# ewrfcas/MVSFormer

Hardware: AMD Instinct MI355X
Metric: depth maps/sec @1536x1152 N=5 D=192 (higher is better)
Workload: dtype f32

## Files before the change

mvsformer_amd/csrc/conv3d_x3_small.hip:

```cpp
#include <stdlib.h>

#include "conv_common.h"
#include "split3.h"

namespace {
using namespace mvsconv;
using mvsx3::bf16x8;
using mvsx3::mfma6;
using mvsx3::Split3;
using mvsx3::split3;

#ifndef SMALL_PF
#define SMALL_PF 4
#endif
constexpr int PF = SMALL_PF;

struct SmallArgs {
    const float* x;
    const bf16x8* wp;
    const float* scale;
    const float* shift;
    const float* residual;
    float* y;
    int B, Cin, Cout, Di, Hi, Wi, Do, Ho, Wo, stride, relu;
    int tiles_w, items;
};

__host__ __device__ inline int steps_of(int nblocks) { return (nblocks + 3) >> 2; }
__host__ __device__ inline int ntap(int p) { return p ? 2 : 1; }
__host__ __device__ inline void dtap(int p, int j, int* k, int* off) {
    if (!p) { *k = 1; *off = 0; }
    else if (j == 0) { *k = 2; *off = 0; }
    else { *k = 0; *off = 1; }
}
__host__ __device__ inline int deconv_class_step0(int KQ, int cls) {
    int s = 0;
    for (int c = 0; c < cls; ++c) s += steps_of(ntap(c >> 2) * ntap((c >> 1) & 1) * ntap(c & 1) * KQ);
    return s;
}
__host__ __device__ inline int deconv_total_steps(int KQ) { return deconv_class_step0(KQ, 8); }

__global__ void small_pack_kernel(const float* __restrict__ w, int Cin, int Cout, int transposed, bf16x8* __restrict__ out, int total) {
    const int idx = blockIdx.x * blockDim.x + threadIdx.x;
    if (idx >= total) return;
    const int KQ = Cin / 8;
    const int lane = idx & 63, term = (idx >> 6) % 3, gstep = idx / 192;
    const int n = lane & 15, kb = lane >> 4;
    bf16x8 v;
    if (!transposed) {
        const int STEPS = steps_of(27 * KQ), ct = gstep / STEPS, step = gstep % STEPS;
        const int q = 4 * step + kb, co = ct * 16 + n;
#pragma unroll
        for (int e = 0; e < 8; ++e) {
            float f = 0.0f;
            if (q < 27 * KQ && co < Cout) f = w[((size_t)co * Cin + (q % KQ) * 8 + e) * 27 + q / KQ];
            v[e] = mvsx3::split3_term(f, term);
        }
    } else {
        const int TOTAL = deconv_total_steps(KQ), ct = gstep / TOTAL;
        int rem = gstep % TOTAL, cls = 0;
        while (cls < 7 && rem >= deconv_class_step0(KQ, cls + 1) - deconv_class_step0(KQ, cls)) {
            rem -= deconv_class_step0(KQ, cls + 1) - deconv_class_step0(KQ, cls);
            ++cls;
        }
        const int pd = cls >> 2, ph = (cls >> 1) & 1, pw = cls & 1;
        const int nh = ntap(ph), nw = ntap(pw), nt = ntap(pd) * nh * nw;
        const int q = 4 * rem + kb, co = ct * 16 + n;
        int kd = 0, kh = 0, kw = 0, o;
        if (q < nt * KQ) {
            const int t = q / KQ;
            dtap(pd, t / (nh * nw), &kd, &o);
            dtap(ph, (t / nw) % nh, &kh, &o);
            dtap(pw, t % nw, &kw, &o);
        }
#pragma unroll
        for (int e = 0; e < 8; ++e) {
            float f = 0.0f;
            if (q < nt * KQ && co < Cout) f = w[((size_t)((q % KQ) * 8 + e) * Cout + co) * 27 + (kd * 3 + kh) * 3 + kw];
            v[e] = mvsx3::split3_term(f, term);
        }
    }
    out[idx] = v;
}

struct WFrag { bf16x8 t[3]; };
__device__ __forceinline__ WFrag load_w(const bf16x8* wk) {
    WFrag f;
#pragma unroll
    for (int t = 0; t < 3; ++t) f.t[t] = wk[t * 64];
    return f;
}
struct AFrag { float f[8]; };
__device__ __forceinline__ AFrag load_a(rsrc_t xin, unsigned voff, unsigned plane_bytes) {
    AFrag a;
#pragma unroll
    for (int e = 0; e < 8; ++e) a.f[e] = buf_load(xin, voff, (unsigned)e * plane_bytes);
    return a;
}
__device__ __forceinline__ f32x4 step_mfma(const AFrag& a, const WFrag& w, f32x4 c) {
    const Split3 s = split3(a.f);
    return mfma6(s.h, s.m, s.l, w.t[0], w.t[1], w.t[2], c);
}

template <bool TRANSPOSED, int KS>
__global__ __launch_bounds__(256) void x3_small_kernel(const SmallArgs a) {
    const int lane = threadIdx.x & 63;
    const int wave = (int)__builtin_amdgcn_readfirstlane(threadIdx.x >> 6);
    const int item = KS == 1 ? blockIdx.x * 4 + wave : blockIdx.x;
    const int ks = KS == 1 ? 0 : wave;
    if (item >= a.items) return;
    __shared__ f32x4 red[KS == 1 ? 1 : 2 * 4 * 64];
    const int m = lane & 15, kb = lane >> 4;
    const int KQ = a.Cin >> 3, kq_shift = 31 - __builtin_clz(KQ);
    const int CT = (a.Cout + 15) >> 4;
    int r = item;
    const int wt = r % a.tiles_w; r /= a.tiles_w;
    const int oh = r % a.Ho; r /= a.Ho;
    const int od = r % a.Do; r /= a.Do;
    const int ct = r % CT, b = r / CT;
    const size_t HWi = (size_t)a.Hi * a.Wi, DHWi = (size_t)a.Di * HWi, HWo = (size_t)a.Ho * a.Wo;
    const rsrc_t xin = make_rsrc(a.x + (size_t)b * a.Cin * DHWi, (unsigned)((size_t)a.Cin * DHWi * 4));
    const unsigned plane_bytes = (unsigned)(DHWi * 4);
    const int co = ct * 16 + m;
    const float sc = (a.scale && co < a.Cout) ? a.scale[co] : 1.0f, sh = (a.shift && co < a.Cout) ? a.shift[co] : 0.0f;
    auto act = [&](float v) {
        v = a.scale ? fmaf(v, sc, sh) : v + sh;
        return a.relu ? fmaxf(v, 0.0f) : v;
    };

    if constexpr (!TRANSPOSED) {
        const int S = a.stride, nblk = 27 * KQ, nsteps = steps_of(nblk);
        const bf16x8* wk = a.wp + (size_t)ct * nsteps * 192 + lane;
        const int ow = wt * 16 + m;
        const int zb = od * S - 1, yb = oh * S - 1, xb = ow * S - 1;
        auto a_off = [&](int s) -> unsigned {
            const int q = 4 * s + kb, t = q >> kq_shift, oct = q & (KQ - 1);
            const int kd = t / 9, kh = (t / 3) % 3, kw = t % 3;
            const int z = zb + kd, y = yb + kh, x = xb + kw;
            const bool ok = q < nblk && ow < a.Wo && (unsigned)z < (unsigned)a.Di && (unsigned)y < (unsigned)a.Hi && (unsigned)x < (unsigned)a.Wi;
            return ok ? ((((unsigned)(oct * 8) * (unsigned)a.Di + (unsigned)z) * (unsigned)a.Hi + (unsigned)y) * (unsigned)a.Wi + (unsigned)x) * 4u : OOB;
        };
        f32x4 acc = {0.f, 0.f, 0.f, 0.f};
        AFrag ar[PF];
        WFrag wr[PF];
#pragma unroll
        for (int i = 0; i < PF; ++i)
            if (ks + i * KS < nsteps) {
                ar[i] = load_a(xin, a_off(ks + i * KS), plane_bytes);
                wr[i] = load_w(wk + (size_t)(ks + i * KS) * 192);
            }
        for (int s0 = ks; s0 < nsteps; s0 += PF * KS) {
#pragma unroll
            for (int i = 0; i < PF; ++i) {
                const int s = s0 + i * KS;
                if (s < nsteps) {
                    acc = step_mfma(ar[i], wr[i], acc);
                    if (s + PF * KS < nsteps) {
                        ar[i] = load_a(xin, a_off(s + PF * KS), plane_bytes);
                        wr[i] = load_w(wk + (size_t)(s + PF * KS) * 192);
                    }
                }
            }
        }
        if constexpr (KS > 1) {
            red[wave * 64 + lane] = acc;
            __syncthreads();
            if (wave != 0) return;
            acc = ((red[lane] + red[64 + lane]) + red[128 + lane]) + red[192 + lane];
        }
        const int ow0 = wt * 16 + kb * 4;
        if (co < a.Cout && ow0 < a.Wo) {
            const size_t o = ((size_t)(b * a.Cout + co) * a.Do + od) * HWo + (size_t)oh * a.Wo + ow0;
            f32x4 v;
#pragma unroll
            for (int i = 0; i < 4; ++i) v[i] = act(acc[i]);
            if ((a.Wo & 3) == 0) {
                if (a.residual) v += *reinterpret_cast<const f32x4*>(a.residual + o);
                *reinterpret_cast<f32x4*>(a.y + o) = v;
            } else {
#pragma unroll
                for (int i = 0; i < 4; ++i)
                    if (ow0 + i < a.Wo) a.y[o + i] = a.residual ? v[i] + a.residual[o + i] : v[i];
            }
        }
    } else {
        const int pd = od & 1, ph = oh & 1, id0 = od >> 1, ih0 = oh >> 1;
        const int iw = wt * 16 + m;
        const int nd = ntap(pd), nh = ntap(ph);
        const int TOTAL = deconv_total_steps(KQ);
        f32x4 acc[2];
#pragma unroll
        for (int pw = 0; pw < 2; ++pw) {
            const int nw = ntap(pw), nblk = nd * nh * nw * KQ, nsteps = steps_of(nblk);
            const int cls = pd * 4 + ph * 2 + pw;
            const bf16x8* wk = a.wp + ((size_t)ct * TOTAL + deconv_class_step0(KQ, cls)) * 192 + lane;
            auto a_off = [&](int s) -> unsigned {
                const int q = 4 * s + kb, t = q >> kq_shift, oct = q & (KQ - 1);
                const int td = t / (nh * nw), th = (t / nw) % nh, tw = t % nw;
                const int z = id0 + (pd ? td : 0), y = ih0 + (ph ? th : 0), x = iw + (pw ? tw : 0);
                const bool ok = q < nblk && z < a.Di && y < a.Hi && x < a.Wi;
                return ok ? ((((unsigned)(oct * 8) * (unsigned)a.Di + (unsigned)z) * (unsigned)a.Hi + (unsigned)y) * (unsigned)a.Wi + (unsigned)x) * 4u : OOB;
            };
            f32x4 c = {0.f, 0.f, 0.f, 0.f};
            AFrag ar[PF];
            WFrag wr[PF];
#pragma unroll
            for (int i = 0; i < PF; ++i)
                if (ks + i * KS < nsteps) {
                    ar[i] = load_a(xin, a_off(ks + i * KS), plane_bytes);
                    wr[i] = load_w(wk + (size_t)(ks + i * KS) * 192);
                }
            for (int s0 = ks; s0 < nsteps; s0 += PF * KS) {
#pragma unroll
                for (int i = 0; i < PF; ++i) {
                    const int s = s0 + i * KS;
                    if (s < nsteps) {
                        c = step_mfma(ar[i], wr[i], c);
                        if (s + PF * KS < nsteps) {
                            ar[i] = load_a(xin, a_off(s + PF * KS), plane_bytes);
                            wr[i] = load_w(wk + (size_t)(s + PF * KS) * 192);
                        }
                    }
                }
            }
            acc[pw] = c;
        }
        if constexpr (KS > 1) {
            red[wave * 64 + lane] = acc[0];
            red[256 + wave * 64 + lane] = acc[1];
            __syncthreads();
            if (wave != 0) return;
            acc[0] = ((red[lane] + red[64 + lane]) + red[128 + lane]) + red[192 + lane];
            acc[1] = ((red[256 + lane] + red[320 + lane]) + red[384 + lane]) + red[448 + lane];
        }
        const int ow0 = 2 * (wt * 16 + kb * 4);
        if (co < a.Cout && ow0 < a.Wo) {
            const size_t o = ((size_t)(b * a.Cout + co) * a.Do + od) * HWo + (size_t)oh * a.Wo + ow0;
            float v[8];
#pragma unroll
            for (int i = 0; i < 4; ++i) {
                v[2 * i] = act(acc[0][i]);
                v[2 * i + 1] = act(acc[1][i]);
            }
            if ((a.Wi & 1) == 0) {
                const bool second = ow0 + 4 < a.Wo;
                if (a.residual) {
                    const f32x4 r0 = *reinterpret_cast<const f32x4*>(a.residual + o);
#pragma unroll
                    for (int i = 0; i < 4; ++i) v[i] += r0[i];
                    if (second) {
                        const f32x4 r1 = *reinterpret_cast<const f32x4*>(a.residual + o + 4);
#pragma unroll
                        for (int i = 0; i < 4; ++i) v[4 + i] += r1[i];
                    }
                }
                *reinterpret_cast<f32x4*>(a.y + o) = f32x4{v[0], v[1], v[2], v[3]};
                if (second) *reinterpret_cast<f32x4*>(a.y + o + 4) = f32x4{v[4], v[5], v[6], v[7]};
            } else {
#pragma unroll
                for (int i = 0; i < 8; ++i)
                    if (ow0 + i < a.Wo) a.y[o + i] = a.residual ? v[i] + a.residual[o + i] : v[i];
            }
        }
    }
}

bool small_ok(int Cin, int Cout, int stride, int transposed) {
    if (Cin != 8 && Cin != 16 && Cin != 32 && Cin != 64) return false;
    if (Cout < 8 || Cout > 64 || (Cout & 7)) return false;
    return transposed ? stride == 2 : (stride == 1 || stride == 2);
}

}

extern "C" int mvs_conv3d_small_supported(int Cin, int Cout, int stride, int transposed) { return small_ok(Cin, Cout, stride, transposed) ? 1 : 0; }

extern "C" int64_t mvs_conv3d_small_packed_bytes(int Cin, int Cout, int stride, int transposed) {
    if (!small_ok(Cin, Cout, stride, transposed)) return 0;
    const int KQ = Cin / 8, CT = (Cout + 15) / 16;
    return (int64_t)CT * (transposed ? deconv_total_steps(KQ) : steps_of(27 * KQ)) * 3 * 64 * 16;
}

extern "C" int mvs_conv3d_small_pack_weights(const float* w, int Cin, int Cout, int stride, int transposed, void* wpacked, mvs_stream_t stream) {
    MVS_REQUIRE(w && wpacked, "mvs_conv3d_small_pack_weights: null pointer");
    MVS_REQUIRE(small_ok(Cin, Cout, stride, transposed), "mvs_conv3d_small_pack_weights: Cin=%d Cout=%d stride=%d transposed=%d is not built", Cin, Cout,
                stride, transposed);
    const int total = (int)(mvs_conv3d_small_packed_bytes(Cin, Cout, stride, transposed) / 16);
    hipLaunchKernelGGL(small_pack_kernel, dim3((total + 255) / 256), dim3(256), 0, MVS_STREAM(stream), w, Cin, Cout, transposed, static_cast<bf16x8*>(wpacked), total);
    return mvs::finish_launch("mvs_conv3d_small_pack_weights");
}

extern "C" int mvs_conv3d_small_fwd(const float* x, const void* wpacked, const float* scale, const float* shift, const float* residual, float* y,
                                    int B, int Cin, int Cout, int D, int H, int W, int stride, int transposed, int relu, mvs_stream_t stream) {
    MVS_REQUIRE(x && wpacked && y, "mvs_conv3d_small_fwd: null pointer");
    MVS_REQUIRE(small_ok(Cin, Cout, stride, transposed), "mvs_conv3d_small_fwd: Cin=%d Cout=%d stride=%d transposed=%d is not built", Cin, Cout, stride,
                transposed);
    MVS_REQUIRE(B >= 1 && D >= 1 && H >= 1 && W >= 1, "mvs_conv3d_small_fwd: bad shape B=%d D=%d H=%d W=%d", B, D, H, W);
    MVS_REQUIRE(!scale || shift, "mvs_conv3d_small_fwd: scale without shift");
    MVS_REQUIRE((int64_t)Cin * D * H * W * 4 < ((int64_t)1 << 31), "mvs_conv3d_small_fwd: one sample's input exceeds the 2 GiB buffer window");
    SmallArgs a;
    a.x = x; a.wp = static_cast<const bf16x8*>(wpacked); a.scale = scale; a.shift = shift; a.residual = residual; a.y = y;
    a.B = B; a.Cin = Cin; a.Cout = Cout; a.Di = D; a.Hi = H; a.Wi = W; a.stride = stride; a.relu = relu;
    if (transposed) {
        a.Do = 2 * D; a.Ho = 2 * H; a.Wo = 2 * W;
        a.tiles_w = mvs::ceil_div(W, 16);
    } else {
        a.Do = (D - 1) / stride + 1; a.Ho = (H - 1) / stride + 1; a.Wo = (W - 1) / stride + 1;
        a.tiles_w = mvs::ceil_div(a.Wo, 16);
    }
    const int64_t items = (int64_t)B * ((Cout + 15) / 16) * a.Do * a.Ho * a.tiles_w;
    MVS_REQUIRE(items < ((int64_t)1 << 31), "mvs_conv3d_small_fwd: too many work items");
    a.items = (int)items;
    const int KQ = Cin / 8, nsteps = transposed ? steps_of(8 * KQ) : steps_of(27 * KQ);
    static const char* env = mvs::env_str("MVS_SMALL_KSPLIT");
    const bool split = env ? atoi(env) != 0 : (nsteps >= 16 && items <= 16384);
    if (split) {
        const dim3 grid((unsigned)items);
        if (transposed) hipLaunchKernelGGL((x3_small_kernel<true, 4>), grid, dim3(256), 0, MVS_STREAM(stream), a);
        else hipLaunchKernelGGL((x3_small_kernel<false, 4>), grid, dim3(256), 0, MVS_STREAM(stream), a);
    } else {
        const dim3 grid((unsigned)((items + 3) / 4));
        if (transposed) hipLaunchKernelGGL((x3_small_kernel<true, 1>), grid, dim3(256), 0, MVS_STREAM(stream), a);
        else hipLaunchKernelGGL((x3_small_kernel<false, 1>), grid, dim3(256), 0, MVS_STREAM(stream), a);
    }
    return mvs::finish_launch("mvs_conv3d_small_fwd");
}
```

mvsformer_amd/module.py:

```python
from __future__ import annotations

from typing import NamedTuple, Optional, Tuple

import torch
import torch.nn as nn

from . import ops, switches as sw
from ._lib import MvsHipError
from .switches import SMALL_MAX_WORK, _parse_small_limit


def _f32c(t: torch.Tensor) -> torch.Tensor:
    return t.detach().to(torch.float32).contiguous()


def _bn_fold(bn: nn.modules.batchnorm._BatchNorm) -> Tuple[torch.Tensor, torch.Tensor]:
    var = bn.running_var.detach().to(torch.float32)
    mean = bn.running_mean.detach().to(torch.float32)
    g = bn.weight.detach().to(torch.float32) if bn.weight is not None else torch.ones_like(var)
    b = bn.bias.detach().to(torch.float32) if bn.bias is not None else torch.zeros_like(var)
    scale = g / torch.sqrt(var + bn.eps)
    return scale.contiguous(), (b - mean * scale).contiguous()


def _versions(*mods: Optional[nn.Module]) -> tuple:
    return (ops.weights_epoch(),) + tuple((t.data_ptr(), t._version) for m in mods if m is not None for t in list(m.parameters()) + list(m.buffers()))


def _publish_cache() -> None:
    if torch.cuda.is_available():
        torch.cuda.current_stream().synchronize()


def autocast_bf16() -> bool:
    if sw.flag("MVS_TRAIN_BF16"):
        return True
    try:
        if hasattr(torch, "get_autocast_dtype"):
            return torch.is_autocast_enabled("cuda") and torch.get_autocast_dtype("cuda") == torch.bfloat16
        return torch.is_autocast_enabled() and torch.get_autocast_gpu_dtype() == torch.bfloat16
    except Exception:
        return False


def _multi_use(t, link=None):
    if link is None and hasattr(t, "_mvs_bn"):
        del t._mvs_bn
    return t


def _skip_links(x, n=3):
    from . import autograd as ag
    if x.dtype == torch.bfloat16 and ag._fused_layers() and sw.flag("MVS_TRAIN_SKIPLINK"):
        return tuple(ag.SkipLink() for _ in range(n))
    return (None,) * n


def _train_conv_bn_act(x, conv, bn, relu, residual, transposed_sd=None, take=None, give=None):
    from . import autograd as ag
    if x.dtype == torch.bfloat16:
        if conv.bias is not None or bn is None:
            raise MvsHipError("bf16 training layer without BatchNorm / with bias is not built")
        fused = 1 if sw.flag("MVS_BN_FUSED_STATS") else 0
        pk = ag.packed_of(conv)
        if ag._fused_layers() and not ag._bn_synced(bn):
            if transposed_sd is None:
                s = tuple(conv.stride)
                return ag.LayerBf16Fn.apply(x, ag.route_of(conv), bn.weight, bn.bias, residual, bn, bool(relu), 0, (s[0], s[1]), 1, pk, take, give)
            return ag.LayerBf16Fn.apply(x, ag.route_of(conv), bn.weight, bn.bias, residual, bn, bool(relu), 1, (transposed_sd, 2), 1, pk, take, give)
        if take is not None:
            _multi_use(x)
        if transposed_sd is None:
            s = tuple(conv.stride)
            out = ag.ConvBf16Fn.apply(x, ag.route_of(conv), (s[0], s[1]), fused, pk)
        else:
            out = ag.DeconvBf16Fn.apply(x, ag.route_of(conv), transposed_sd, fused, pk)
        y, sums = out if fused else (out, None)
        return ag.BnActBf16Fn.apply(y, bn.weight, bn.bias, residual, bn, bool(relu), 1, sums)
    if transposed_sd is None:
        s = tuple(conv.stride)
        y = ag.ConvFn.apply(x, conv.weight, (s[0], s[1]))
    else:
        y = ag.DeconvFn.apply(x, conv.weight, transposed_sd)
    if conv.bias is not None:
        raise MvsHipError("training-mode conv with bias (bn=False) is not built")
    if bn is None:
        raise MvsHipError("training-mode layer without BatchNorm is not built")
    return ag.BnActFn.apply(y, bn.weight, bn.bias, residual, bn, bool(relu))


_SMALL_LIMITS = _parse_small_limit(sw.text("MVS_CONV_SMALL_MAX_WORK"))
_WINDOW = 1 << 31


class RouteSwitches(NamedTuple):
    min_voxels: int = sw.TABLE["MVS_CONV_X3_MIN_VOXELS"].default
    small_limit: Tuple[int, int] = SMALL_MAX_WORK
    conv_x3: str = "1"
    conv_wino: Optional[str] = None
    tail: str = "x3"
    fuse_prob: bool = True


def route_switches() -> RouteSwitches:
    return RouteSwitches(sw.integer("MVS_CONV_X3_MIN_VOXELS"), _SMALL_LIMITS, sw.text("MVS_CONV_X3"), sw.text("MVS_CONV_WINO"),
                         sw.text("MVS_TAIL"), sw.flag("MVS_FUSE_PROB"))


def _small_limit(rs: RouteSwitches, transposed: bool) -> int:
    return 0 if rs.conv_x3 == "0" else rs.small_limit[1 if transposed else 0]


def conv_route(cin, cout, stride, in_shape, forms, rs: RouteSwitches, wino_ok: bool = False) -> str:
    D, H, W = in_shape
    if "x3" in forms and rs.conv_x3 != "0" and D * (H // stride[1]) * (W // stride[1]) >= rs.min_voxels and cin * D * H * W * 4 < _WINDOW:
        return "x3"
    if "small" in forms and ((D - 1) // stride[0] + 1) * ((H - 1) // stride[1] + 1) * ((W - 1) // stride[1] + 1) * cin * cout <= _small_limit(rs, False):
        return "small"
    if "wino" in forms and wino_ok:
        return "wino"
    return "fp32"


def deconv_route(cin, cout, sd, in_shape, forms, rs: RouteSwitches, x3_ok: bool = False, residual_bytes: int = 0) -> str:
    D, H, W = in_shape
    if sd == 1:
        if cout >= 16 and rs.conv_x3 != "0" and x3_ok and W % 2 == 0 and 4 * D * H * W >= rs.min_voxels \
                and cin * D * H * W * 4 < _WINDOW and residual_bytes < 2 * _WINDOW:
            return "x3"
        return "fp32"
    if "small" in forms and D * H * W * cin * cout <= _small_limit(rs, True):
        return "small"
    return "fp32"


def tail_route(cin, cout, sd, in_shape, rs: RouteSwitches, skip_bytes: int = 0) -> str:
    D, H, W = in_shape
    if not (cout == 8 and sd == 1 and W % 4 == 0 and rs.fuse_prob):
        return "unfused"
    if cin == 16 and rs.conv_x3 != "0" and rs.tail == "x3" and 4 * D * H * W >= rs.min_voxels and skip_bytes < _WINDOW:
        return "tail_x3"
    return "tail_fp32"


class _EvalLayer:

    _key = None

    @staticmethod
    def check(conv) -> Tuple[int, int]:
        s = tuple(conv.stride)
        if isinstance(conv, nn.ConvTranspose3d):
            if tuple(conv.kernel_size) != (3, 3, 3) or tuple(conv.padding) != (1, 1, 1) or conv.groups != 1:
                raise MvsHipError("Deconv3d: only kernel 3, padding 1, groups 1 is built (got %s)" % conv)
            if (s, tuple(conv.output_padding)) not in (((2, 2, 2), (1, 1, 1)), ((1, 2, 2), (0, 1, 1))):
                raise MvsHipError("Deconv3d: stride %s / output_padding %s is not built" % (s, tuple(conv.output_padding)))
        elif tuple(conv.kernel_size) != (3, 3, 3) or tuple(conv.padding) != (1, 1, 1) or tuple(conv.dilation) != (1, 1, 1) or conv.groups != 1:
            raise MvsHipError("Conv3d: only kernel 3, padding 1, dilation 1, groups 1 is built (got %s)" % conv)
        elif s not in ((1, 1, 1), (2, 2, 2), (1, 2, 2)):
            raise MvsHipError("Conv3d: stride %s is not built" % (s,))
        return s[0], s[1]

    def _sync(self, conv, bn, rs: RouteSwitches) -> None:
        key = (_versions(conv, bn), rs.conv_x3, rs.conv_wino, rs.small_limit)
        if key == self._key:
            return
        self.transposed = isinstance(conv, nn.ConvTranspose3d)
        self.cin, self.cout, self.stride = cin, cout, s = conv.in_channels, conv.out_channels, self.check(conv)
        w = _f32c(conv.weight)
        self.forms = forms = {"fp32": ops.conv3d_pack(w, self.transposed, s[0])}
        self.x3_ok = self.transposed and s[0] == 1 and ops.deconv3d_x3_supported(cin, cout, 1)
        if self.transposed:
            if s[0] == 2 and cout >= 16 and _small_limit(rs, True) > 0 and ops.conv3d_small_supported(cin, cout, 2, True):
                forms["small"] = ops.conv3d_small_pack(w, 2, True)
        else:
            if s == (1, 1) and cin % 4 == 0 and cout % 16 == 0 and cout <= 64 and rs.conv_wino == "1":
                forms["wino"] = ops.conv3d_wino_pack(w)
            if rs.conv_x3 != "0" and ops.conv3d_x3_supported(cin, cout, s) \
                    and not (rs.conv_x3 == "strided" and s[1] == 1) and not (rs.conv_x3 == "s1" and s[1] == 2):
                forms["x3"] = ops.conv3d_x3_pack(w, s)
            if s[0] == s[1] and _small_limit(rs, False) > 0 and ops.conv3d_small_supported(cin, cout, s[0], False):
                forms["small"] = ops.conv3d_small_pack(w, s[0], False)
        self.scale, self.shift = _bn_fold(bn) if bn is not None else (None, _f32c(conv.bias) if conv.bias is not None else None)
        _publish_cache()
        self._key = key

    def _late_form(self, name: str, conv, pack):
        if name not in self.forms:
            self.forms[name] = pack(_f32c(conv.weight))
            _publish_cache()
        return self.forms[name]

    def run(self, conv, bn, relu: bool, x, residual, rs: RouteSwitches):
        self._sync(conv, bn, rs)
        cin, cout, stride, f, scale, shift = self.cin, self.cout, self.stride, self.forms, self.scale, self.shift
        if not self.transposed:
            route = conv_route(cin, cout, stride, x.shape[2:], f, rs, "wino" in f and ops.conv3d_wino_supported(cin, cout, *x.shape[2:]))
            if route == "x3":
                return ops.conv3d_x3(x, f["x3"], cin, cout, stride, scale, shift, residual, relu=relu)
            if route == "small":
                return ops.conv3d_small(x, f["small"], cin, cout, stride[0], False, scale, shift, residual, relu=relu)
            if route == "wino":
                return ops.conv3d_wino(x, f["wino"], cin, cout, scale, shift, residual, relu=relu)
            return ops.conv3d(x, f["fp32"], cin, cout, stride, scale, shift, residual, relu=relu, tag="conv3d_%dto%d_s%d%d" % (cin, cout, *stride))
        sd = stride[0]
        route = deconv_route(cin, cout, sd, x.shape[2:], f, rs, self.x3_ok, 0 if residual is None else residual[0].numel() * 4)
        if route == "x3":
            return ops.deconv3d_x3(x, self._late_form("x3", conv, lambda w: ops.deconv3d_x3_pack(w, sd)), cin, cout, sd, scale, shift, residual, relu=relu)
        if route == "small":
            return ops.conv3d_small(x, f["small"], cin, cout, 2, True, scale, shift, residual, relu=relu)
        return ops.deconv3d(x, f["fp32"], cin, cout, sd, scale, shift, residual, relu=relu, tag="deconv3d_%dto%d_s%d" % (cin, cout, sd))

    def run_tail(self, conv, bn, x, skip, w1, b1, rs: RouteSwitches):
        self._sync(conv, bn, rs)
        route = tail_route(self.cin, self.cout, self.stride[0], x.shape[2:], rs, skip.numel() * 4)
        if route == "tail_x3":
            return ops.tail_x3(x, self._late_form("tail_x3", conv, ops.tail_x3_pack), self.scale, self.shift, skip, w1, b1, relu=True)
        if route == "tail_fp32":
            return ops.deconv3d_prob1(x, self.forms["fp32"], self.cin, self.scale, self.shift, skip, w1, b1, relu=True)
        return ops.prob1(self.run(conv, bn, True, x, skip, rs), w1, b1).squeeze(1)


class Conv3d(nn.Module):

    def __init__(self, in_channels, out_channels, kernel_size=3, stride=1, relu=True, bn=True, bn_momentum=0.1, init_method="xavier", **kwargs):
        super().__init__()
        self.out_channels = out_channels
        self.kernel_size = kernel_size
        self.conv = nn.Conv3d(in_channels, out_channels, kernel_size, stride=stride, bias=(not bn), **kwargs)
        self.bn = nn.BatchNorm3d(out_channels, momentum=bn_momentum) if bn else None
        self.relu = relu
        self._layer = _EvalLayer()

    def forward(self, x, residual: Optional[torch.Tensor] = None, take=None, _rs: Optional[RouteSwitches] = None):
        if self.training:
            return _train_conv_bn_act(x, self.conv, self.bn, self.relu, residual, take=take)
        return self._layer.run(self.conv, self.bn, self.relu, x, residual, _rs or route_switches())


class Deconv3d(nn.Module):

    def __init__(self, in_channels, out_channels, kernel_size=3, stride=1, relu=True, bn=True, bn_momentum=0.1, init_method="xavier", **kwargs):
        super().__init__()
        self.out_channels = out_channels
        self.conv = nn.ConvTranspose3d(in_channels, out_channels, kernel_size, stride=stride, bias=(not bn), **kwargs)
        self.bn = nn.BatchNorm3d(out_channels, momentum=bn_momentum) if bn else None
        self.relu = relu
        self._layer = _EvalLayer()

    def forward(self, x, residual: Optional[torch.Tensor] = None, give=None, _rs: Optional[RouteSwitches] = None):
        if self.training:
            _EvalLayer.check(self.conv)
            return _train_conv_bn_act(x, self.conv, self.bn, self.relu, residual, transposed_sd=self.conv.stride[0], give=give)
        return self._layer.run(self.conv, self.bn, self.relu, x, residual, _rs or route_switches())


class ConvBnReLU(nn.Module):

    def __init__(self, in_channels: int, out_channels: int, kernel_size: int = 3, stride: int = 1, pad: int = 1, dilation: int = 1):
        super().__init__()
        self.conv = nn.Conv2d(in_channels, out_channels, kernel_size, stride=stride, padding=pad, dilation=dilation, bias=False)
        self.bn = nn.BatchNorm2d(out_channels)

    def forward(self, x):
        raise MvsHipError("ConvBnReLU is a parameter holder; the fused visibility CNN runs through StageNet (mvs_vis_fwd)")


def pack_vis_params(vis: nn.Sequential) -> torch.Tensor:
    c0, c1, c2, c3 = vis[0], vis[1], vis[2], vis[3]
    shapes = [tuple(c.conv.weight.shape) for c in (c0, c1, c2)] + [tuple(c3.weight.shape)]
    if shapes != [(16, 1, 3, 3), (16, 16, 3, 3), (8, 16, 3, 3), (1, 8, 1, 1)]:
        raise MvsHipError("vis CNN has unexpected shapes %s" % (shapes,))
    parts = []
    for c in (c0, c1, c2):
        w = _f32c(c.conv.weight)
        parts.append(w.permute(1, 2, 3, 0).reshape(-1))
        s, b = _bn_fold(c.bn)
        parts += [s, b]
    parts += [_f32c(c3.weight).reshape(-1), _f32c(c3.bias).reshape(-1)]
    out = torch.cat(parts).contiguous()
    assert out.numel() == ops.VIS_PARAM_FLOATS
    return out


def _volume_input(net, x: torch.Tensor, strided: int, bf16_ok: bool):
    if not isinstance(net.inner, nn.Identity):
        raise MvsHipError("%s: in_channels != base channels (1x1x1 'inner' conv) is not built" % type(net).__name__)
    pre16 = bf16_ok and x.dtype == torch.bfloat16
    if not pre16:
        x = x.to(torch.float32)
    x = x if x.is_contiguous() else x.contiguous()
    dhw = tuple(x.shape[1:4] if pre16 else x.shape[2:])[-strided:]
    if any(n % 8 for n in dhw):
        raise MvsHipError("%s needs %s divisible by 8 (three stride-2 levels), got %s" % (type(net).__name__, ("H, W", "D, H, W")[strided - 2], dhw))
    return x, pre16


class CostRegNet(nn.Module):

    def __init__(self, in_channels, base_channels, last_layer=True):
        super().__init__()
        self.last_layer = last_layer
        b = base_channels
        self.conv1 = Conv3d(in_channels, b * 2, stride=2, padding=1)
        self.conv2 = Conv3d(b * 2, b * 2, padding=1)
        self.conv3 = Conv3d(b * 2, b * 4, stride=2, padding=1)
        self.conv4 = Conv3d(b * 4, b * 4, padding=1)
        self.conv5 = Conv3d(b * 4, b * 8, stride=2, padding=1)
        self.conv6 = Conv3d(b * 8, b * 8, padding=1)
        self.conv7 = Deconv3d(b * 8, b * 4, stride=2, padding=1, output_padding=1)
        self.conv9 = Deconv3d(b * 4, b * 2, stride=2, padding=1, output_padding=1)
        self.conv11 = Deconv3d(b * 2, b * 1, stride=2, padding=1, output_padding=1)
        if in_channels != base_channels:
            self.inner = nn.Conv3d(in_channels, base_channels, 1, 1)
        else:
            self.inner = nn.Identity()
        if self.last_layer:
            self.prob = nn.Conv3d(base_channels, 1, 3, stride=1, padding=1, bias=False)

    def features(self, x: torch.Tensor) -> torch.Tensor:
        x, pre16 = _volume_input(self, x, 3, self.training)
        if self.training and autocast_bf16() and not pre16:
            from . import autograd as ag
            x = ag.ToBf16Fn.apply(x)
        if not self.training:
            rs = route_switches()
            c2 = self.conv2(self.conv1(x, _rs=rs), _rs=rs)
            c4 = self.conv4(self.conv3(c2, _rs=rs), _rs=rs)
            y = self.conv7(self.conv6(self.conv5(c4, _rs=rs), _rs=rs), residual=c4, _rs=rs)
            return self.conv11(self.conv9(y, residual=c2, _rs=rs), residual=x, _rs=rs)
        l0, l2, l4 = _skip_links(x)
        c2 = _multi_use(self.conv2(self.conv1(x, take=l0)), l2)
        c4 = _multi_use(self.conv4(self.conv3(c2, take=l2)), l4)
        y = self.conv6(self.conv5(c4, take=l4))
        y = self.conv7(y, residual=c4, give=l4)
        y = self.conv9(y, residual=c2, give=l2)
        return _multi_use(self.conv11(y, residual=x, give=l0))

    def forward(self, x):
        y = self.features(x)
        if self.last_layer:
            if self.training:
                from . import autograd as ag
                pk = ag.packed_of(self.prob) if y.dtype == torch.bfloat16 else None
                if pk is not None and ag._fused_layers():
                    y = ag.Select0Bf16Fn.apply(ag.ConvBf16Fn.apply(y, ag.route_of(self.prob), (1, 1), 0, pk, 8)).unsqueeze(1)
                else:
                    w8 = torch.nn.functional.pad(self.prob.weight, (0, 0, 0, 0, 0, 0, 0, 0, 0, 7))
                    if y.dtype == torch.bfloat16:
                        y = ag.FromBf16Fn.apply(ag.ConvBf16Fn.apply(y, w8, (1, 1)))[:, :1]
                    else:
                        y = ag.ConvFn.apply(y, w8, (1, 1))[:, :1]
            else:
                y = ops.prob3(y, _f32c(self.prob.weight)).unsqueeze(1)
        return y


def _deconv_seq(cin, cout):
    return nn.Sequential(
        nn.ConvTranspose3d(cin, cout, kernel_size=3, padding=1, output_padding=(0, 1, 1), stride=(1, 2, 2), bias=False),
        nn.BatchNorm3d(cout), nn.ReLU(inplace=True))


class CostRegNet3D(nn.Module):

    def __init__(self, in_channels, base_channel=8):
        super().__init__()
        b = base_channel
        self.conv1 = Conv3d(in_channels, b * 2, kernel_size=3, stride=(1, 2, 2), padding=1)
        self.conv2 = Conv3d(b * 2, b * 2, padding=1)
        self.conv3 = Conv3d(b * 2, b * 4, kernel_size=3, stride=(1, 2, 2), padding=1)
        self.conv4 = Conv3d(b * 4, b * 4, padding=1)
        self.conv5 = Conv3d(b * 4, b * 8, kernel_size=3, stride=(1, 2, 2), padding=1)
        self.conv6 = Conv3d(b * 8, b * 8, padding=1)
        self.conv7 = _deconv_seq(b * 8, b * 4)
        self.conv9 = _deconv_seq(b * 4, b * 2)
        self.conv11 = _deconv_seq(b * 2, b)
        if in_channels != base_channel:
            self.inner = nn.Conv3d(in_channels, base_channel, 1, 1)
        else:
            self.inner = nn.Identity()
        self.prob = nn.Conv3d(base_channel, 1, 1, stride=1, padding=0)
        self._layers = {name: _EvalLayer() for name in ("conv7", "conv9", "conv11")}

    def _up(self, name: str, x, residual, give=None, _rs: Optional[RouteSwitches] = None):
        seq = getattr(self, name)
        if self.training:
            _EvalLayer.check(seq[0])
            return _train_conv_bn_act(x, seq[0], seq[1], True, residual, transposed_sd=seq[0].stride[0], give=give)
        return self._layers[name].run(seq[0], seq[1], True, x, residual, _rs or route_switches())

    def logits(self, x: torch.Tensor) -> torch.Tensor:
        rs = None if self.training else route_switches()
        y, skip = self._trunk(x, rs)
        if self.training:
            return ops.prob1(self._up("conv11", y, skip), *self.prob_params()).squeeze(1)
        return self._layers["conv11"].run_tail(self.conv11[0], self.conv11[1], y, skip, *self.prob_params(), rs)

    def _trunk(self, x: torch.Tensor, rs: Optional[RouteSwitches]):
        x, _ = _volume_input(self, x, 2, False)
        c2 = self.conv2(self.conv1(x, _rs=rs), _rs=rs)
        c4 = self.conv4(self.conv3(c2, _rs=rs), _rs=rs)
        y = self.conv6(self.conv5(c4, _rs=rs), _rs=rs)
        y = self._up("conv7", y, c4, _rs=rs)
        return self._up("conv9", y, c2, _rs=rs), x

    def features(self, x: torch.Tensor) -> torch.Tensor:
        if not self.training:
            rs = route_switches()
            y, skip = self._trunk(x, rs)
            return self._up("conv11", y, skip, _rs=rs)
        x, pre16 = _volume_input(self, x, 2, True)
        if autocast_bf16() and not pre16:
            from . import autograd as ag
            x = ag.ToBf16Fn.apply(x)
        l0, l2, l4 = _skip_links(x)
        c2 = _multi_use(self.conv2(self.conv1(x, take=l0)), l2)
        c4 = _multi_use(self.conv4(self.conv3(c2, take=l2)), l4)
        y = self.conv6(self.conv5(c4, take=l4))
        y = self._up("conv7", y, c4, l4)
        y = self._up("conv9", y, c2, l2)
        return _multi_use(self._up("conv11", y, x, l0))

    def prob_params(self):
        return _f32c(self.prob.weight).reshape(-1), _f32c(self.prob.bias).reshape(-1)

    def forward(self, x):
        y = self.features(x)
        if self.training:
            from . import autograd as ag
            if y.dtype == torch.bfloat16:
                if ag._fused_layers():
                    return ag.HeadBf16Fn.apply(y, self.prob.weight, self.prob.bias, False).unsqueeze(1)
                y = ag.FromBf16Fn.apply(y)
            return ag.Prob1Fn.apply(y, self.prob.weight, self.prob.bias)
        w, b = self.prob_params()
        return ops.prob1(y, w, b)


def depth_regression(p, depth_values):
    if depth_values.dim() > 2 and depth_values.shape != p.shape:
        depth_values = depth_values.expand_as(p)
    return ops.depth_regression(p.to(torch.float32).contiguous(), depth_values.to(torch.float32).contiguous())


def conf_regression(p, n=4):
    return ops.conf_regression(p.detach().to(torch.float32).contiguous(), n)


def init_inverse_range(cur_depth, ndepths, device, dtype, H, W):
    return ops.init_inverse_range(cur_depth.to(torch.float32).contiguous(), ndepths, H, W)


def init_range(cur_depth, ndepths, device, dtype, H, W):
    return ops.init_range(cur_depth.to(torch.float32).contiguous(), ndepths, H, W)


def schedule_range(cur_depth, ndepth, depth_inteval_pixel, H, W):
    return ops.schedule_range(cur_depth.to(torch.float32).contiguous(), depth_inteval_pixel.to(torch.float32).contiguous(), ndepth, 1.0, H, W)


def schedule_inverse_range(depth, depth_hypo, ndepths, split_itv, H, W):
    return ops.schedule_inverse_range(depth.to(torch.float32).contiguous(), depth_hypo.to(torch.float32).contiguous(),
                                      ndepths, float(split_itv), H, W)
```

mvsformer_amd/switches.py:

```python
from __future__ import annotations

import os
from typing import NamedTuple, Optional, Tuple


class Switch(NamedTuple):
    name: str
    default: object
    kind: str
    meaning: str
    read: str = "call"
    values: Optional[Tuple[str, ...]] = None


_ROWS = (
    Switch("MVS_CONV_X3", "1", "str", "`0` = regularizer layers on the fp32 instead of the bf16 matrix cores (3-term split form, DESIGN §4.7; also turns the "
           "small-volume split form off); `strided` / `s1` = split form for the stride-(1,2,2) / the stride-1 convolutions only (diagnostics)", "pack"),
    Switch("MVS_CONV_X3_MIN_VOXELS", 40 * 1024, "int", "output voxels from which a layer uses the split form; below, it keeps the fp32 kernel"),
    Switch("MVS_CONV_SMALL_MAX_WORK", None, "str", "`conv,deconv` or one value for both: voxels x Cin x Cout up to which the small-volume split form "
           "serves a layer (unset: 16777216,8388608; `0` = never)", "import"),
    Switch("MVS_CONV_WINO", None, "str", "`1` = Winograd fp32 convolution for the stride-1 layers in eval (opt-in: the split form is as fast); the training "
           "forward uses it unless `0`", "pack"),
    Switch("MVS_FUSE_PROB", True, "on", "`0` = conv11 and the 1x1x1 `prob` as two launches"),
    Switch("MVS_TAIL", "x3", "str", "anything but `x3` (say `fp32`) = the fused conv11 + `prob` tail on the fp32 instead of the bf16 matrix cores"),
    Switch("MVS_CV_FAST", False, "off", "`1` = sweeps with one reciprocal + hardware exp2/log2 instead of the reference's op order with IEEE divisions"),
    Switch("MVS_CV_STORE_MAX_MB", 160.0, "float", "size limit of a coarse stage's stored correlation; 0 = always recompute"),
    Switch("MVS_CV_STORE_BANDS", 1, "int", "row bands in which a stage whose store is larger may run the stored-correlation sweeps (bit-identical)"),
    Switch("MVS_CV_TILED", False, "off", "`1` = the LDS-tiled sweeps instead of the direct-gather sweeps (DESIGN §4.2c; ignored by `StageNet.forward_bank`)"),
    Switch("MVS_VIS", None, "str", "visibility CNN on the bf16 matrix cores in split form (`x3`) / Winograd fp32 MFMA (`wino`) / all-VALU (`valu`); "
           "unset: `x3`, or `valu` with `MVS_VIS_WINO=0`", "pack", ("x3", "wino", "valu")),
    Switch("MVS_VIS_WINO", True, "on", "`0` = `MVS_VIS=valu` where `MVS_VIS` is unset", "pack"),
    Switch("MVS_TRANSPOSE_MULTI", True, "on", "`0` = one NCHW -> NHWC transpose launch per stage instead of one for the cascade"),
    Switch("MVS_FPN_X3", "1", "str", "`0` = the FPN's full-resolution layers on the fp32 matrix cores; `strip` = the decoder's last level as the split-form "
           "strip kernel (`csrc/fpn_x3.hip`) instead of the contraction-first kernel (`csrc/fpn_cp.hip`)", "pack"),
    Switch("MVS_FPN_V2_TAIL", True, "on", "`0` = `FPNDecoderV2`'s full-resolution tail through the generic split-form GEMMs (up map written, added, read back) "
           "instead of the fused kernel (`csrc/fpn_v2_tail.hip`)", "pack"),
    Switch("MVS_VIT_PACKED", True, "on", "`0` = the ViT with operands split inside every GEMM block instead of pre-split"),
    Switch("MVS_VIT_FLASH", True, "on", "`0` = materialized attention in every block of the unpacked eval ViT (`MVS_VIT_PACKED=0`)"),
    Switch("MVS_VIT_TRAIN_FLASH", True, "on", "`0` = ViT training (`\"fix\": false`) with materialized attention instead of `csrc/vit_flash_train.hip`"),
    Switch("MVS_TRAIN_BF16", False, "off", "`1` = bf16 regularizer in training without an autocast context"),
    Switch("MVS_TRAIN_FUSED", True, "on", "`0` = separate conv / BatchNorm autograd nodes, per-layer weight packing and fp32 heads instead of the fused layer nodes"),
    Switch("MVS_TRAIN_SKIPLINK", True, "on", "`0` = autograd adds a skip tensor's two gradients (instead of the strided layer's data-gradient epilogue)"),
    Switch("MVS_TRAIN_WGRAD_GROUP", True, "on", "`0` = every layer runs its own weight gradient instead of one grouped launch per kernel instance"),
    Switch("MVS_TRAIN_WGRAD_SCOPE", "cascade", "str", "`stage` = one weight-gradient group per stage instead of one for the cascade"),
    Switch("MVS_BN_FUSED_STATS", False, "off", "`1` = the unfused bf16 training convolution takes the batch statistics in its epilogue (measured slower)"),
    Switch("MVS_VIS_BF16", True, "on", "`0` = the visibility CNN stays fp32 under autocast"),
    Switch("MVS_VIS_PER_VIEW", False, "off", "`1` = the training visibility CNN runs view by view instead of batched over the source views"),
    Switch("MVS_CV_BWD", "own", "str", "scatter of the cost-volume backward: per-wavefront LDS windows with owner election / block-shared window with "
           "LDS atomics / global atomics (DESIGN §4.5)", "call", ("own", "lds", "direct")),
    Switch("MVS_CV_BWD_WINDOW", None, "str", "`log2(WX),WY` texel window of the cost-volume backward (unset: `5,20` for `own`, `6,24` for `lds`)"),
    Switch("MVS_TAG_SHAPES", False, "off", "`1` = the grouped weight gradient's timer tag carries its shape"),
    Switch("MVS_HIP_LIB", None, "str", "path of another build of `libmvs_hip.so` (`make -C mvsformer_amd/csrc variants` or `exp`)", "import"),
)
TABLE = {s.name: s for s in _ROWS}


def _get(name: str, kinds) -> Tuple[Switch, Optional[str]]:
    row = TABLE.get(name)
    if row is None or row.kind not in kinds:
        raise KeyError("%s is not a%s switch of mvsformer_amd.switches.TABLE" % (name, "" if row is None else " " + "/".join(kinds)))
    return row, os.environ.get(name)


def flag(name: str) -> bool:
    row, v = _get(name, ("on", "off"))
    return v != "0" if row.kind == "on" else v == "1"


def integer(name: str) -> int:
    row, v = _get(name, ("int",))
    return int(row.default if v is None else v)


def number(name: str) -> float:
    row, v = _get(name, ("float",))
    return float(row.default if v is None else v)


def text(name: str, error=ValueError) -> Optional[str]:
    row, v = _get(name, ("str",))
    if v is None:
        return row.default
    if row.values is not None and v not in row.values:
        raise error("%s must be one of %s, not %r" % (name, ", ".join(row.values), v))
    return v


SMALL_MAX_WORK = (16 << 20, 8 << 20)


def _parse_small_limit(text) -> Tuple[int, int]:
    if not text:
        return SMALL_MAX_WORK
    try:
        v = [int(t) for t in text.split(",")]
    except ValueError:
        v = []
    if len(v) == 1:
        v = v * 2
    if len(v) != 2 or min(v) < 0:
        raise ValueError("MVS_CONV_SMALL_MAX_WORK must be 'conv,deconv' or one non-negative integer, got %r" % (text,))
    return v[0], v[1]


def readme_table() -> str:
    def shown(s):
        if s.default is None:
            return "unset"
        if s.kind in ("on", "off"):
            return "1" if s.default else "0"
        return "%g" % s.default if s.kind == "float" else str(s.default)
    head = "| name | default | meaning | read |\n|---|---|---|---|\n"
    return head + "".join("| `%s` | %s | %s | %s |\n" % (s.name, shown(s), s.meaning, s.read) for s in _ROWS)
```

Measured before the change: 271.1.

## Add paired-parity deconv kernel for Cin16/Cout8 and widen small-conv routing

Adds a dedicated stride-2 transposed-conv kernel for Cin=16, Cout=8 that packs two W-parities into one 16-wide MFMA tile, so all eight output octants share input fragments and the 8-channel output no longer wastes half of each MFMA column. It has its own weight packing layout. The routing sends this shape to the new kernel above a minimum work size, and raises the small-conv work limit for the Cin8→Cout16 stride-2 conv. The cost is extra code paths, a shuffle-based interleaved store, and a possible routing shift toward kernels that may be slower at some sizes.

```diff
diff --git a/mvsformer_amd/csrc/conv3d_x3_small.hip b/mvsformer_amd/csrc/conv3d_x3_small.hip
--- a/mvsformer_amd/csrc/conv3d_x3_small.hip
+++ b/mvsformer_amd/csrc/conv3d_x3_small.hip
@@ -40,6 +40,10 @@
 }
 __host__ __device__ inline int deconv_total_steps(int KQ) { return deconv_class_step0(KQ, 8); }
 
+constexpr int PAIR_STEPS = 9;
+__host__ __device__ inline int pair_step0(int cls) { return cls == 0 ? 0 : (cls == 1 ? 1 : (cls == 2 ? 3 : 5)); }
+__host__ __device__ inline bool pair_form(int Cin, int Cout, int transposed) { return transposed && Cin == 16 && Cout == 8; }
+
 __global__ void small_pack_kernel(const float* __restrict__ w, int Cin, int Cout, int transposed, bf16x8* __restrict__ out, int total) {
     const int idx = blockIdx.x * blockDim.x + threadIdx.x;
     if (idx >= total) return;
@@ -79,6 +83,27 @@
             if (q < nt * KQ && co < Cout) f = w[((size_t)((q % KQ) * 8 + e) * Cout + co) * 27 + (kd * 3 + kh) * 3 + kw];
             v[e] = mvsx3::split3_term(f, term);
         }
+    }
+    out[idx] = v;
+}
+
+__global__ void small_pair_pack_kernel(const float* __restrict__ w, bf16x8* __restrict__ out) {
+    const int idx = blockIdx.x * blockDim.x + threadIdx.x;
+    if (idx >= PAIR_STEPS * 192) return;
+    const int lane = idx & 63, term = (idx >> 6) % 3, gstep = idx / 192;
+    const int n = lane & 15, kb = lane >> 4, pw = n >> 3, co = n & 7, tw = kb >> 1, oct = kb & 1;
+    const int cls = gstep < 1 ? 0 : (gstep < 3 ? 1 : (gstep < 5 ? 2 : 3)), j = gstep - pair_step0(cls);
+    const int pd = cls >> 1, ph = cls & 1;
+    const int td = pd ? (ph ? j >> 1 : j) : 0, th = ph ? (pd ? j & 1 : j) : 0;
+    int kd, kh, kw, o;
+    dtap(pd, td, &kd, &o);
+    dtap(ph, th, &kh, &o);
+    dtap(pw, tw, &kw, &o);
+    bf16x8 v;
+#pragma unroll
+    for (int e = 0; e < 8; ++e) {
+        const float f = (pw == 0 && tw == 1) ? 0.0f : w[((size_t)(oct * 8 + e) * 8 + co) * 27 + (kd * 3 + kh) * 3 + kw];
+        v[e] = mvsx3::split3_term(f, term);
     }
     out[idx] = v;
 }
@@ -265,6 +290,86 @@
     }
 }
 
+__global__ __launch_bounds__(256) void x3_small_pair_kernel(const SmallArgs a) {
+    const int lane = threadIdx.x & 63;
+    const int wave = (int)__builtin_amdgcn_readfirstlane(threadIdx.x >> 6);
+    const int item = blockIdx.x * 4 + wave;
+    if (item >= a.items) return;
+    const int m = lane & 15, kb = lane >> 4;
+    int r = item;
+    const int wt = r % a.tiles_w; r /= a.tiles_w;
+    const int ih = r % a.Hi; r /= a.Hi;
+    const int id = r % a.Di, b = r / a.Di;
+    const size_t HWi = (size_t)a.Hi * a.Wi, DHWi = (size_t)a.Di * HWi, HWo = (size_t)a.Ho * a.Wo;
+    const rsrc_t xin = make_rsrc(a.x + (size_t)b * 16 * DHWi, (unsigned)(16 * DHWi * 4));
+    const unsigned plane_bytes = (unsigned)(DHWi * 4);
+    const bf16x8* wk = a.wp + lane;
+    WFrag w0[4];
+#pragma unroll
+    for (int c = 0; c < 4; ++c) w0[c] = load_w(wk + (size_t)pair_step0(c) * 192);
+    const int tw = kb >> 1, oct = kb & 1, x = wt * 16 + m + tw;
+    AFrag ar[4];
+#pragma unroll
+    for (int j = 0; j < 4; ++j) {
+        const int z = id + (j >> 1), y = ih + (j & 1);
+        const bool ok = z < a.Di && y < a.Hi && x < a.Wi;
+        ar[j] = load_a(xin, ok ? ((((unsigned)(oct * 8) * (unsigned)a.Di + (unsigned)z) * (unsigned)a.Hi + (unsigned)y) * (unsigned)a.Wi + (unsigned)x) * 4u : OOB,
+                       plane_bytes);
+    }
+    f32x4 acc[4];
+#pragma unroll
+    for (int c = 0; c < 4; ++c) acc[c] = f32x4{0.f, 0.f, 0.f, 0.f};
+    {
+        const Split3 s = split3(ar[0].f);
+#pragma unroll
+        for (int c = 0; c < 4; ++c) acc[c] = mfma6(s.h, s.m, s.l, w0[c].t[0], w0[c].t[1], w0[c].t[2], acc[c]);
+    }
+    {
+        const WFrag w1 = load_w(wk + (size_t)(pair_step0(1) + 1) * 192), w3 = load_w(wk + (size_t)(pair_step0(3) + 1) * 192);
+        const Split3 s = split3(ar[1].f);
+        acc[1] = mfma6(s.h, s.m, s.l, w1.t[0], w1.t[1], w1.t[2], acc[1]);
+        acc[3] = mfma6(s.h, s.m, s.l, w3.t[0], w3.t[1], w3.t[2], acc[3]);
+    }
+    {
+        const WFrag w2 = load_w(wk + (size_t)(pair_step0(2) + 1) * 192), w3 = load_w(wk + (size_t)(pair_step0(3) + 2) * 192);
+        const Split3 s = split3(ar[2].f);
+        acc[2] = mfma6(s.h, s.m, s.l, w2.t[0], w2.t[1], w2.t[2], acc[2]);
+        acc[3] = mfma6(s.h, s.m, s.l, w3.t[0], w3.t[1], w3.t[2], acc[3]);
+    }
+    {
+        const WFrag w3 = load_w(wk + (size_t)(pair_step0(3) + 3) * 192);
+        const Split3 s = split3(ar[3].f);
+        acc[3] = mfma6(s.h, s.m, s.l, w3.t[0], w3.t[1], w3.t[2], acc[3]);
+    }
+    const int pw = m >> 3, co = m & 7;
+    const float sc = a.scale ? a.scale[co] : 1.0f, sh = a.shift ? a.shift[co] : 0.0f;
+    const int ow = 2 * (wt * 16 + kb * 4) + 4 * pw;
+    const bool vec = (a.Wi & 1) == 0;
+#pragma unroll
+    for (int c = 0; c < 4; ++c) {
+        float v[4];
+#pragma unroll
+        for (int i = 0; i < 4; ++i) {
+            const float t = a.scale ? fmaf(acc[c][i], sc, sh) : acc[c][i] + sh;
+            v[i] = a.relu ? fmaxf(t, 0.0f) : t;
+        }
+        const float g0 = __shfl_xor(pw ? v[0] : v[2], 8), g1 = __shfl_xor(pw ? v[1] : v[3], 8);
+        f32x4 q = pw ? f32x4{g0, v[2], g1, v[3]} : f32x4{v[0], g0, v[1], g1};
+        if (ow < a.Wo) {
+            const int od = 2 * id + (c >> 1), oh = 2 * ih + (c & 1);
+            const size_t o = ((size_t)(b * 8 + co) * a.Do + od) * HWo + (size_t)oh * a.Wo + ow;
+            if (vec) {
+                if (a.residual) q += *reinterpret_cast<const f32x4*>(a.residual + o);
+                *reinterpret_cast<f32x4*>(a.y + o) = q;
+            } else {
+#pragma unroll
+                for (int i = 0; i < 4; ++i)
+                    if (ow + i < a.Wo) a.y[o + i] = a.residual ? q[i] + a.residual[o + i] : q[i];
+            }
+        }
+    }
+}
+
 bool small_ok(int Cin, int Cout, int stride, int transposed) {
     if (Cin != 8 && Cin != 16 && Cin != 32 && Cin != 64) return false;
     if (Cout < 8 || Cout > 64 || (Cout & 7)) return false;
@@ -277,6 +382,7 @@
 
 extern "C" int64_t mvs_conv3d_small_packed_bytes(int Cin, int Cout, int stride, int transposed) {
     if (!small_ok(Cin, Cout, stride, transposed)) return 0;
+    if (pair_form(Cin, Cout, transposed)) return (int64_t)PAIR_STEPS * 3 * 64 * 16;
     const int KQ = Cin / 8, CT = (Cout + 15) / 16;
     return (int64_t)CT * (transposed ? deconv_total_steps(KQ) : steps_of(27 * KQ)) * 3 * 64 * 16;
 }
@@ -286,6 +392,10 @@
     MVS_REQUIRE(small_ok(Cin, Cout, stride, transposed), "mvs_conv3d_small_pack_weights: Cin=%d Cout=%d stride=%d transposed=%d is not built", Cin, Cout,
                 stride, transposed);
     const int total = (int)(mvs_conv3d_small_packed_bytes(Cin, Cout, stride, transposed) / 16);
+    if (pair_form(Cin, Cout, transposed)) {
+        hipLaunchKernelGGL(small_pair_pack_kernel, dim3((total + 255) / 256), dim3(256), 0, MVS_STREAM(stream), w, static_cast<bf16x8*>(wpacked));
+        return mvs::finish_launch("mvs_conv3d_small_pack_weights");
+    }
     hipLaunchKernelGGL(small_pack_kernel, dim3((total + 255) / 256), dim3(256), 0, MVS_STREAM(stream), w, Cin, Cout, transposed, static_cast<bf16x8*>(wpacked), total);
     return mvs::finish_launch("mvs_conv3d_small_pack_weights");
 }
@@ -308,6 +418,13 @@
         a.Do = (D - 1) / stride + 1; a.Ho = (H - 1) / stride + 1; a.Wo = (W - 1) / stride + 1;
         a.tiles_w = mvs::ceil_div(a.Wo, 16);
     }
+    if (pair_form(Cin, Cout, transposed)) {
+        const int64_t n = (int64_t)B * D * H * a.tiles_w;
+        MVS_REQUIRE(n < ((int64_t)1 << 31), "mvs_conv3d_small_fwd: too many work items");
+        a.items = (int)n;
+        hipLaunchKernelGGL(x3_small_pair_kernel, dim3((unsigned)((n + 3) / 4)), dim3(256), 0, MVS_STREAM(stream), a);
+        return mvs::finish_launch("mvs_conv3d_small_fwd");
+    }
     const int64_t items = (int64_t)B * ((Cout + 15) / 16) * a.Do * a.Ho * a.tiles_w;
     MVS_REQUIRE(items < ((int64_t)1 << 31), "mvs_conv3d_small_fwd: too many work items");
     a.items = (int)items;
diff --git a/mvsformer_amd/module.py b/mvsformer_amd/module.py
--- a/mvsformer_amd/module.py
+++ b/mvsformer_amd/module.py
@@ -7,7 +7,7 @@
 
 from . import ops, switches as sw
 from ._lib import MvsHipError
-from .switches import SMALL_MAX_WORK, _parse_small_limit
+from .switches import SMALL_MAX_WORK, SMALL_PAIR_MIN_WORK, SMALL_WIDE_MAX_WORK, _parse_small_limit
 
 
 def _f32c(t: torch.Tensor) -> torch.Tensor:
@@ -107,15 +107,19 @@
                          sw.text("MVS_TAIL"), sw.flag("MVS_FUSE_PROB"))
 
 
-def _small_limit(rs: RouteSwitches, transposed: bool) -> int:
-    return 0 if rs.conv_x3 == "0" else rs.small_limit[1 if transposed else 0]
+def _small_limit(rs: RouteSwitches, transposed: bool, wide: bool = False) -> int:
+    if rs.conv_x3 == "0":
+        return 0
+    i = 1 if transposed else 0
+    return SMALL_WIDE_MAX_WORK if wide and rs.small_limit[i] == SMALL_MAX_WORK[i] else rs.small_limit[i]
 
 
 def conv_route(cin, cout, stride, in_shape, forms, rs: RouteSwitches, wino_ok: bool = False) -> str:
     D, H, W = in_shape
     if "x3" in forms and rs.conv_x3 != "0" and D * (H // stride[1]) * (W // stride[1]) >= rs.min_voxels and cin * D * H * W * 4 < _WINDOW:
         return "x3"
-    if "small" in forms and ((D - 1) // stride[0] + 1) * ((H - 1) // stride[1] + 1) * ((W - 1) // stride[1] + 1) * cin * cout <= _small_limit(rs, False):
+    wide = (cin, cout, tuple(stride)) == (8, 16, (2, 2))
+    if "small" in forms and ((D - 1) // stride[0] + 1) * ((H - 1) // stride[1] + 1) * ((W - 1) // stride[1] + 1) * cin * cout <= _small_limit(rs, False, wide):
         return "small"
     if "wino" in forms and wino_ok:
         return "wino"
@@ -129,7 +133,10 @@
                 and cin * D * H * W * 4 < _WINDOW and residual_bytes < 2 * _WINDOW:
             return "x3"
         return "fp32"
-    if "small" in forms and D * H * W * cin * cout <= _small_limit(rs, True):
+    work = D * H * W * cin * cout
+    if (cin, cout) == (16, 8):
+        return "small" if "small" in forms and SMALL_PAIR_MIN_WORK < work <= _small_limit(rs, True, True) else "fp32"
+    if "small" in forms and work <= _small_limit(rs, True):
         return "small"
     return "fp32"
 
@@ -171,7 +178,7 @@
         self.forms = forms = {"fp32": ops.conv3d_pack(w, self.transposed, s[0])}
         self.x3_ok = self.transposed and s[0] == 1 and ops.deconv3d_x3_supported(cin, cout, 1)
         if self.transposed:
-            if s[0] == 2 and cout >= 16 and _small_limit(rs, True) > 0 and ops.conv3d_small_supported(cin, cout, 2, True):
+            if s[0] == 2 and (cout >= 16 or (cin, cout) == (16, 8)) and _small_limit(rs, True) > 0 and ops.conv3d_small_supported(cin, cout, 2, True):
                 forms["small"] = ops.conv3d_small_pack(w, 2, True)
         else:
             if s == (1, 1) and cin % 4 == 0 and cout % 16 == 0 and cout <= 64 and rs.conv_wino == "1":
diff --git a/mvsformer_amd/switches.py b/mvsformer_amd/switches.py
--- a/mvsformer_amd/switches.py
+++ b/mvsformer_amd/switches.py
@@ -87,6 +87,8 @@
 
 
 SMALL_MAX_WORK = (16 << 20, 8 << 20)
+SMALL_WIDE_MAX_WORK = 32 << 20
+SMALL_PAIR_MIN_WORK = SMALL_MAX_WORK[1]
 
 
 def _parse_small_limit(text) -> Tuple[int, int]:
```

Result: no change. 271.4, median of 4 (+0.1%).
